# tyfeld/MMaDA-Parallel

Hardware: AMD Instinct MI355X
Metric: images/sec (512x512, 64 img + 128 text steps) MMaDA-Parallel-A 8B (higher is better)
Workload: dtype bf16

## Files before the change

mmada_parallel_amd/build.py:

```python
from __future__ import annotations

import os
import shutil
import subprocess
import sys
from concurrent.futures import ThreadPoolExecutor

HERE = os.path.dirname(os.path.abspath(__file__))
ROOT = os.path.dirname(HERE)
CSRC = os.path.join(HERE, "csrc")
OBJ = os.path.join(CSRC, "_obj")
LIB_NAME = "libmmada_mi355x.so"
LIB_PATH = os.path.join(HERE, LIB_NAME)
SOURCES = ["gemm.hip", "gemm8.hip", "attention.hip", "elementwise.hip", "sampler.hip", "vq_decoder.hip", "graph.hip", "tp_comm.hip", "probe.hip", "api.hip"]
HEADERS = ["exports.map", "common.h", "kernels.h", "gemm_epilogue.h", "handle.h", "attention.h", os.path.join("..", "..", "include", "mmada_mi355x.h")]
FLAGS = ["--offload-arch=gfx950", "-O3", "-std=c++17", "-fPIC", "-fvisibility=hidden", "-fvisibility-inlines-hidden", "-Wno-unused-result"]
UNIT_FLAGS = {"attention.hip": ["-fno-slp-vectorize", "-fno-honor-nans"]}


def _hipcc() -> str:
    for cand in (os.environ.get("HIPCC"), shutil.which("hipcc"), "/opt/rocm/bin/hipcc"):
        if cand and os.path.exists(cand):
            return cand
    raise RuntimeError("hipcc not found (set HIPCC or install ROCm)")


def needs_build() -> bool:
    if not os.path.exists(LIB_PATH):
        return True
    t = os.path.getmtime(LIB_PATH)
    deps = [os.path.join(CSRC, s) for s in SOURCES + HEADERS]
    return any(os.path.getmtime(d) > t for d in deps)


def _run(cmd):
    proc = subprocess.run(cmd, capture_output=True, text=True)
    if proc.returncode != 0:
        raise RuntimeError("hipcc failed:\n" + " ".join(cmd) + "\n" + proc.stdout + proc.stderr)
    return proc.stdout


def compile_objects(out_dir: str, extra_flags=(), force: bool = False, verbose: bool = False, jobs: int = 0):
    os.makedirs(out_dir, exist_ok=True)
    hdr_t = max(os.path.getmtime(os.path.join(CSRC, h)) for h in HEADERS)
    todo, objs = [], []
    for src in SOURCES:
        obj = os.path.join(out_dir, src.replace(".hip", ".o"))
        objs.append(obj)
        sp = os.path.join(CSRC, src)
        if force or not os.path.exists(obj) or os.path.getmtime(obj) < max(hdr_t, os.path.getmtime(sp)):
            todo.append([_hipcc(), *FLAGS, *UNIT_FLAGS.get(src, []), *extra_flags, "-c", sp, "-o", obj])
    if verbose:
        for c in todo:
            print(" ".join(c))
    with ThreadPoolExecutor(max_workers=jobs or min(len(todo) or 1, os.cpu_count() or 4)) as ex:
        list(ex.map(_run, todo))
    return objs


def verify_isa() -> None:
    tools = os.path.join(ROOT, "tools")
    if not os.path.exists(os.path.join(tools, "isa_check.py")):
        print("build: tools/isa_check.py not found, compiled-code checks skipped", file=sys.stderr)
        return
    if tools not in sys.path:
        sys.path.insert(0, tools)
    import isa_check

    with ThreadPoolExecutor(max_workers=2) as ex:
        asm8, asma = ex.map(isa_check.device_asm, ["gemm8.hip", "attention.hip"])
    errors = []
    errors += isa_check.check_gemm8(asm8)[1]
    errors += isa_check.check_gemm8_rowstat(asm8)[1]
    errors += isa_check.check_attention(asma)[1]
    if errors:
        raise RuntimeError("compiled-code checks failed (tools/isa_check.py):\n" + "\n".join(errors))


def build(force: bool = False, verbose: bool = False, verify: bool = False) -> str:
    if not force and not needs_build():
        return LIB_PATH
    with ThreadPoolExecutor(max_workers=2) as ex:
        chk = ex.submit(verify_isa) if verify else None
        objs = compile_objects(OBJ, force=force, verbose=verbose)
        _run([_hipcc(), "--offload-arch=gfx950", "-shared", "-fPIC", "-Wl,--version-script=" + os.path.join(CSRC, "exports.map"), *objs,
              "-o", LIB_PATH + ".tmp"])
        if chk is not None:
            try:
                chk.result()
            except Exception:
                for o in objs + [LIB_PATH + ".tmp"]:
                    if os.path.exists(o):
                        os.remove(o)
                raise
    os.replace(LIB_PATH + ".tmp", LIB_PATH)
    return LIB_PATH


if __name__ == "__main__":
    print(build(force="--force" in sys.argv, verbose=True, verify="--verify" in sys.argv))
```

mmada_parallel_amd/csrc/api.hip:

```cpp
#include <algorithm>
#include <cstdarg>
#include <cstdio>
#include <cstdlib>
#include <cstring>
#include <cmath>
#include <utility>
#include <vector>

#include "../../include/mmada_mi355x.h"
#include "handle.h"
#include "gemm_epilogue.h"

static thread_local char g_err[1024] = "";

int mm_fail(const char* fmt, ...) {
    va_list ap;
    va_start(ap, fmt);
    vsnprintf(g_err, sizeof(g_err), fmt, ap);
    va_end(ap);
    return 1;
}

extern "C" {

// ... 146 lines not shown
int mmada_embed(mmada_handle* h, const int64_t* ids, int B, int L, void* stream) {
    if (!h || !ids) return mm_fail("mmada_embed: null argument");
    hipStream_t s = (hipStream_t)stream;
    if (check_bound(h)) return 1;
    if (apply_carve(h, B, L, s)) return 1;
    h->cur_W = 0; h->cur_beg = 0; h->Mcur = h->M;
    h->xn_is_final = false;
    h->xn_is_layer0 = true;
    return launch_embed(ids, h->wte, h->x, B, L, h->Lp, h->cfg.d_model, h->cfg.vocab, s, h->layers[0].attn_norm, h->xn,
                        h->cfg.rms_eps);
}

}

GemmArgs qkv_args(const mmada_handle* h, int layer, int m0, int rows) {
    const int d = h->cfg.d_model;
    GemmArgs g = gemm_bt_args(h->xn + (size_t)m0 * d, h->layers[layer].wqkv, nullptr, rows, (h->hq_l + 2 * h->hkv_l) * 128, d, 0);
    g.m_base = m0;
    g.q = h->q; g.k = h->k; g.vT = h->vT; g.rope_cos = h->rope_cos; g.rope_sin = h->rope_sin;
    g.Lp = h->Lp; g.Lkv = h->Lkv; g.Hq = h->hq_l; g.Hkv = h->hkv_l;
    if (const CacheSlot* cc = h->cc) {
        g.k = cc->K(layer); g.vT = cc->vT(layer); g.Lkv = cc->Lkv;
        g.pos_map = h->cc_pos; g.Lq = h->Lkv; g.q_pos_shift = h->cc_qshift;
    }
    return g;
}

GemmArgs gate_up_args(const mmada_handle* h, int layer, int m0, int rows) {
    const int d = h->cfg.d_model;
    return gemm_bt_args(h->xn + (size_t)m0 * d, h->layers[layer].wgu, h->hbuf + (size_t)m0 * h->f_l, rows, 2 * h->f_l, d, h->f_l);
}

GemmArgs attn_out_args(const mmada_handle* h, int layer, int m0, int rows) {
    const int d = h->cfg.d_model, K = h->hq_l * 128;
    return gemm_bt_args(h->att + (size_t)m0 * K, h->layers[layer].wo, h->y + (size_t)m0 * d, rows, d, K, d);
}

GemmArgs down_args(const mmada_handle* h, int layer, int m0, int rows) {
    const int d = h->cfg.d_model;
    return gemm_bt_args(h->hbuf + (size_t)m0 * h->f_l, h->layers[layer].wdown, h->y + (size_t)m0 * d, rows, d, h->f_l, d);
}

int block_attention(mmada_handle* h, int layer, hipStream_t s, int wbeg, int W) {
    const CacheSlot* cc = h->cc;
    const double rows = W ? (double)h->B * W : (double)h->B * h->L;
    ProfScope p(h, layer, 1, 4.0 * h->hq_l * rows * (cc ? cc->L : h->L) * 128.0, s);
    if (cc)
        return launch_attention(h->q, cc->K(layer), cc->vT(layer), h->att, h->B, h->hq_l, h->hkv_l, cc->L, h->Lp, cc->Lkv, h->Lp,
                                h->hq_l * 128, s, 0, h->Lkv);
    if (W)
        return launch_attention(h->q, h->k, h->vT, h->att, h->B, h->hq_l, h->hkv_l, h->L, wbeg + W, h->Lkv, W, h->hq_l * 128, s,
                                wbeg);
    return launch_attention(h->q, h->k, h->vT, h->att, h->B, h->hq_l, h->hkv_l, h->L, h->Lp, h->Lkv, h->Lp, h->hq_l * 128, s);
}

static int run_blocks(mmada_handle* h, void* stream) {
    for (int i = 0; i < h->cfg.n_layers; ++i)
        if (mmada_attn_partial(h, i, stream) || mmada_mlp_partial(h, i, stream)) return 1;
    return 0;
}

extern "C" {

int mmada_attn_partial(mmada_handle* h, int layer, void* stream) {
    if (!h || h->M == 0) return mm_fail("mmada_attn_partial: call mmada_embed first");
    if (layer < 0 || layer >= h->cfg.n_layers) return mm_fail("mmada_attn_partial: bad layer");
    hipStream_t s = (hipStream_t)stream;
    const int d = h->cfg.d_model;
    if (layer == 0 && h->xn_is_layer0) {
        h->xn_is_layer0 = false;
    } else if (launch_rmsnorm(h->x, h->layers[layer].attn_norm, h->xn, h->M, d, h->cfg.rms_eps, s)) return 1;
    const GemmArgs g = qkv_args(h, layer, 0, h->M);
    const double rows = (double)h->B * h->L;
    {
        ProfScope p(h, layer, 0, 2.0 * rows * g.N * g.K, s);
        if (launch_gemm(EPI_QKV, g, s)) return 1;
    }
    int wbeg = 0, wend = 0, W = 0;
    if (!h->cc && layer == h->cfg.n_layers - 1 && h->win_end > h->win_beg) {
        if (h->win_end > h->L) return mm_fail("forward: consumed rows [%d,%d) exceed L=%d", h->win_beg, h->win_end, h->L);
        wbeg = h->win_beg & ~31;
        wend = std::min((h->win_end + 7) & ~7, h->Lp);
        W = wend - wbeg;
        if (W >= h->Lp) { wbeg = 0; W = 0; }
    }
    if (block_attention(h, layer, s, wbeg, W)) return 1;
    const int Mo = W ? h->B * W : h->M;
    const double orows = W ? (double)h->B * W : rows;
    GemmArgs o = attn_out_args(h, layer, 0, Mo);
    o.resid = h->x; o.ldr = d; o.resid_mod = h->cfg.tp_size; o.resid_rank = h->cfg.tp_rank;
    if (W) { o.rwin = W; o.rlp = h->Lp; o.rbeg = wbeg; }
    {
        ProfScope p(h, layer, 2, 2.0 * orows * o.N * o.K, s);
        if (launch_gemm(EPI_RESID, o, s)) return 1;
    }
    std::swap(h->x, h->y);
    if (W) { h->cur_W = W; h->cur_beg = wbeg; h->Mcur = Mo; }
    return 0;
}

int mmada_mlp_partial(mmada_handle* h, int layer, void* stream) {
    if (!h || h->M == 0) return mm_fail("mmada_mlp_partial: call mmada_embed first");
    if (layer < 0 || layer >= h->cfg.n_layers) return mm_fail("mmada_mlp_partial: bad layer");
    hipStream_t s = (hipStream_t)stream;
    const int d = h->cfg.d_model;
    if (launch_rmsnorm(h->x, h->layers[layer].ff_norm, h->xn, h->Mcur, d, h->cfg.rms_eps, s)) return 1;
    const GemmArgs g = gate_up_args(h, layer, 0, h->Mcur);
    const double rows = h->cur_W ? (double)h->Mcur : (double)h->B * h->L;
    {
        ProfScope p(h, layer, 3, 2.0 * rows * g.N * g.K, s);
        if (launch_gemm(EPI_SWIGLU, g, s)) return 1;
    }
    GemmArgs o = down_args(h, layer, 0, h->Mcur);
    o.resid = h->x; o.ldr = d; o.resid_mod = h->cfg.tp_size; o.resid_rank = h->cfg.tp_rank;
    {
        ProfScope p(h, layer, 4, 2.0 * rows * o.N * o.K, s);
        if (launch_gemm(EPI_RESID, o, s)) return 1;
    }
    std::swap(h->x, h->y);
    return 0;
}

int mmada_profile_begin(mmada_handle* h, int layer) {
    if (!h) return mm_fail("mmada_profile_begin: null handle");
    for (auto& r : h->prof) h->prof_pool.push_back({r.a, r.b});
    h->prof.clear();
    h->prof_layer = layer;
    return 0;
}

int mmada_profile_end(mmada_handle* h, int32_t* count_out, double* ms_out, double* flops_out) {
    if (!h || !count_out || !ms_out || !flops_out) return mm_fail("mmada_profile_end: null argument");
    for (int i = 0; i < 5; ++i) { count_out[i] = 0; ms_out[i] = 0.0; flops_out[i] = 0.0; }
    for (auto& r : h->prof) {
        MM_CHECK_HIP(hipEventSynchronize(r.b));
        float ms = 0.f;
        MM_CHECK_HIP(hipEventElapsedTime(&ms, r.a, r.b));
        count_out[r.kind] += 1; ms_out[r.kind] += ms; flops_out[r.kind] += r.flops;
        h->prof_pool.push_back({r.a, r.b});
    }
    h->prof.clear();
    h->prof_layer = -1;
    return 0;
}

}

static struct {
    std::atomic<int> gemm_config{-2};
    std::atomic<int> gemm_silu_lut{-1};
    std::atomic<int> gemm_short_tiles{-1};
    std::atomic<int> gemm_tile_order{-1};
    std::atomic<int> attention_form{-1};
    std::atomic<int> probe_variant{0};
    std::atomic<int> tp_allow_single_rank{0};
} g_switches;

static int env_int(const char* name, int fallback) {
    const char* e = getenv(name);
    return e ? atoi(e) : fallback;
}
static int env_flag(const char* name) {
    const char* e = getenv(name);
    return e && e[0] == '0' ? 0 : 1;
}

Switches switches() {
    static const Switches env = {env_int("MMADA_GEMM_CFG", -1), env_flag("MMADA_GEMM_SILU_LUT"), env_flag("MMADA_GEMM_SHORT_TILES"),
                                 env_int("MMADA_GEMM_TILE_ORDER", 0), env_int("MMADA_ATTN_FORM", 1), 0, 0};
    const int cfg = g_switches.gemm_config, lut = g_switches.gemm_silu_lut, shrt = g_switches.gemm_short_tiles,
              order = g_switches.gemm_tile_order, form = g_switches.attention_form;
    return {cfg == -2 ? env.gemm_config : cfg, lut < 0 ? env.gemm_silu_lut : lut, shrt < 0 ? env.gemm_short_tiles : shrt,
            order < 0 ? env.gemm_tile_order : order, form < 0 ? env.attention_form : form, g_switches.probe_variant,
            g_switches.tp_allow_single_rank};
}

extern "C" {

int mmada_set_option(const char* name, int value) {
    if (!name) return mm_fail("mmada_set_option: null name");
    static const struct { const char* name; std::atomic<int>* field; bool flag; } table[] = {
        {"gemm_config", &g_switches.gemm_config, false},
        {"gemm_silu_lut", &g_switches.gemm_silu_lut, true},
        {"gemm_short_tiles", &g_switches.gemm_short_tiles, true},
        {"gemm_tile_order", &g_switches.gemm_tile_order, false},
        {"attention_form", &g_switches.attention_form, false},
        {"probe_variant", &g_switches.probe_variant, false},
        {"tp_allow_single_rank", &g_switches.tp_allow_single_rank, true},
    };
    for (const auto& o : table)
        if (!strcmp(name, o.name)) {
            o.field->store(o.flag ? value != 0 : value);
            return 0;
        }
    return mm_fail("mmada_set_option: unknown option '%s'", name);
}

int mmada_gemm_swiglu_bt(const void* A, const void* W, void* C, int M, int N, int K, void* stream) {
    if (!A || !W || !C || M <= 0 || N <= 0 || K <= 0 || N % 64) return mm_fail("mmada_gemm_swiglu_bt: bad argument");
    return launch_gemm(EPI_SWIGLU, gemm_bt_args((const bf16_t*)A, (const bf16_t*)W, (bf16_t*)C, M, N, K, N / 2), (hipStream_t)stream);
}

int mmada_gemm_plan(int M, int N, int K) { return gemm_plan_code(M, N, K); }
int mmada_attention_plan(int pairs, int groups, int keys) {
    if (pairs <= 0 || groups <= 0 || keys <= 0) return mm_fail("mmada_attention_plan: bad argument"), -1;
    return attention_chunks(pairs, groups, keys);
}

int mmada_probe_f2bf(const float* in, uint16_t* out, int64_t n, void* stream) {
    if (!in || !out || n < 0) return mm_fail("mmada_probe_f2bf: bad argument");
    return launch_f2bf_probe(in, out, (long long)n, (hipStream_t)stream);
}

size_t mmada_mfma_probe_bytes(void) { return (size_t)64 * 8 * 16 * 64 * 16; }

int mmada_mfma_probe(const void* data, void* sink, int iters, int launches, void* stream, double* tflops_out, double* ms_out) {
    if (!data || !sink || iters <= 0 || launches <= 0) return mm_fail("mmada_mfma_probe: bad argument");
    return launch_mfma_probe((const bf16_t*)data, (float*)sink, iters, launches, (hipStream_t)stream, tflops_out, ms_out);
}

void* mmada_stream_ptr(mmada_handle* h) { return h ? (void*)h->x : nullptr; }
size_t mmada_stream_bytes(const mmada_handle* h) { return h ? (size_t)h->Mcur * h->cfg.d_model * 2 : 0; }

int mmada_forward_body(mmada_handle* h, const int64_t* ids, int B, int L, void* stream) {
    if (!h) return mm_fail("mmada_forward_body: null handle");
    if (h->cfg.tp_size != 1 || tp_comm_connected(h)) {
        if (!h->tp)
            return mm_fail("mmada_forward_body: tp_size=%d needs a connected collective (mmada_comm_create + "
                           "mmada_comm_connect_*) or the host-issued all-reduce of the segment API", h->cfg.tp_size);
        if (mmada_embed(h, ids, B, L, stream)) return 1;
        return tp_forward_body(h, (hipStream_t)stream);
    }
    if (mmada_embed(h, ids, B, L, stream)) return 1;
    return run_blocks(h, stream);
}

static void slot_layout(const mmada_handle* h, int B, int L, CacheSlot& c) {
    c.B = B; c.L = L; c.Lp = ceil_to(L, 8); c.Lkv = ceil_to(L, 64);
    c.kv_bytes = align_up((size_t)B * h->hkv_l * c.Lkv * 128 * 2, 256);
    c.layer_stride = 2 * c.kv_bytes;
    c.bytes = (size_t)h->cfg.n_layers * c.layer_stride + align_up((size_t)B * c.Lp * h->cfg.d_model * 2, 256);
}

size_t mmada_cache_bytes(const mmada_handle* h, int B, int L) {
    if (!h || B <= 0 || L <= 0) return 0;
    CacheSlot c;
    slot_layout(h, B, L, c);
    return c.bytes;
}

int mmada_cache_bind(mmada_handle* h, int slot, void* mem, size_t bytes, int B, int L, void* stream) {
    if (!h) return mm_fail("mmada_cache_bind: null handle");
    if (slot < 0 || slot >= MMADA_CACHE_SLOTS) return mm_fail("mmada_cache_bind: slot %d outside [0,%d)", slot, MMADA_CACHE_SLOTS);
    if (!mem) {
        h->slots[slot] = CacheSlot{};
        return 0;
    }
    if (h->cfg.tp_size != 1 && !tp_comm_connected(h))
        return mm_fail("mmada_cache_bind: tp_size=%d needs the library's exchange connected (mmada_comm_create + mmada_comm_connect_*)", h->cfg.tp_size);
    if (B <= 0 || L <= 0 || L > h->cfg.max_seq) return mm_fail("mmada_cache_bind: bad shape B=%d L=%d", B, L);
    if (((uintptr_t)mem) & 255) return mm_fail("mmada_cache_bind: memory must be 256-byte aligned");
    CacheSlot c;
    slot_layout(h, B, L, c);
    if (bytes < c.bytes) return mm_fail("mmada_cache_bind: %zu bytes given, %zu needed", bytes, c.bytes);
    c.mem = (char*)mem;
    MM_CHECK_HIP(hipMemsetAsync(mem, 0, c.bytes, (hipStream_t)stream));
    h->slots[slot] = c;
    return 0;
}

int mmada_forward_cached(mmada_handle* h, int slot, const int64_t* ids, const int32_t* pos, int B, int L, int Tc,
                         int q_pos_from_map, void* stream) {
    if (!h || !ids) return mm_fail("mmada_forward_cached: null argument");
    if (slot < 0 || slot >= MMADA_CACHE_SLOTS || !h->slots[slot].mem) return mm_fail("mmada_forward_cached: slot %d is not bound", slot);
    const CacheSlot& c = h->slots[slot];
    if (c.B != B || c.L != L) return mm_fail("mmada_forward_cached: slot holds B=%d L=%d, call has B=%d L=%d", c.B, c.L, B, L);
    const bool tp = h->cfg.tp_size != 1 || tp_comm_connected(h);
    if (tp && !tp_comm_connected(h)) return mm_fail("mmada_forward_cached: tp_size=%d needs the library's exchange connected", h->cfg.tp_size);
    if (!pos) Tc = L;
    if (Tc <= 0 || Tc > L) return mm_fail("mmada_forward_cached: Tc=%d outside (0,%d]", Tc, L);
    hipStream_t s = (hipStream_t)stream;
    if (check_bound(h)) return 1;
    if (apply_carve(h, B, L, s)) return 1;
    if (pos) {
        h->L = Tc; h->Lp = ceil_to(Tc, 8); h->Lkv = ceil_to(Tc, 64); h->M = B * h->Lp;
        if (launch_expand_pos(pos, h->posmap, B, Tc, h->Lp, L, s)) { h->M = 0; return 1; }
    }
    h->cur_W = 0; h->cur_beg = 0; h->Mcur = h->M;
    h->xn_is_final = false;
    h->xn_is_layer0 = true;
    const int d = h->cfg.d_model;
    if (launch_embed(ids, h->wte, h->x, B, h->L, h->Lp, d, h->cfg.vocab, s, h->layers[0].attn_norm, h->xn, h->cfg.rms_eps)) {
        h->M = 0;
        return 1;
    }
    h->cc = &c;
    h->cc_pos = pos ? h->posmap : nullptr;
    h->cc_qshift = (pos && !q_pos_from_map) ? L - Tc : -1;
    const int rc = tp ? tp_forward_body(h, s) : run_blocks(h, stream);
    h->cc = nullptr; h->cc_pos = nullptr; h->cc_qshift = -1;
    if (rc) { h->M = 0; return 1; }
    bf16_t* xfin = c.xfin(h->cfg.n_layers);
    const bf16_t* fin = tp ? h->xn : h->x;
    h->slots[slot].normalized = tp;
    if (pos) {
        if (launch_scatter_rows(fin, xfin, h->posmap, h->M, h->Lp, c.Lp, d, s)) { h->M = 0; return 1; }
    } else {
        MM_CHECK_HIP(hipMemcpyAsync(xfin, fin, (size_t)h->M * d * 2, hipMemcpyDeviceToDevice, s));
    }
    h->xn_is_final = false;
    h->M = 0;
    return 0;
}

int mmada_cache_head_rows(mmada_handle* h, int slot, const int32_t* rows, int R, int col_begin, int col_end,
                          void* logits_out, void* stream) {
    if (!h || !rows || !logits_out) return mm_fail("mmada_cache_head_rows: null argument");
    if (slot < 0 || slot >= MMADA_CACHE_SLOTS || !h->slots[slot].mem) return mm_fail("mmada_cache_head_rows: slot %d is not bound", slot);
    const CacheSlot& c = h->slots[slot];
    if (R <= 0) return 0;
    if (R > c.B * c.L) return mm_fail("mmada_cache_head_rows: R=%d exceeds B*L=%d", R, c.B * c.L);
    if (col_begin < 0 || col_end > h->cfg.vocab || col_begin >= col_end) return mm_fail("mmada_cache_head_rows: bad column range");
    hipStream_t s = (hipStream_t)stream;
    const int d = h->cfg.d_model;
    bf16_t* xg;
    if (h->M != 0) {
        if ((size_t)R > (size_t)h->B * h->L)
            return mm_fail("mmada_cache_head_rows: %d rows do not fit the resident forward's gather buffer (%d x %d rows); "
                           "ask for fewer rows per call", R, h->B, h->L);
        xg = h->xg;
    } else {
        const Carve cv = carve_for(h, c.B, c.L);
        if (!h->ws || cv.total > h->ws_bytes) return mm_fail("mmada_cache_head_rows: workspace too small (%zu needed)", cv.total);
        xg = (bf16_t*)(h->ws + cv.xg);
    }
    if (c.normalized) {
        if (tp_gather_rows(c.xfin(h->cfg.n_layers), rows, R, c.L, c.Lp, d, c.B * c.L, xg, s)) return 1;
    } else if (launch_rmsnorm_gather(c.xfin(h->cfg.n_layers), h->ln_f, xg, rows, R, c.L, c.Lp, d, h->cfg.rms_eps, s, 0, c.B * c.L))
// ... 195 lines not shown
```

mmada_parallel_amd/csrc/gemm8.hip:

```cpp
#include "gemm_epilogue.h"

namespace {

using namespace gemm_detail;

constexpr int BK = 64;

#define G8_SB() __builtin_amdgcn_sched_barrier(0)
#define G8_BARRIER()                            \
    do {                                        \
        G8_SB();                                \
        asm volatile("s_barrier" ::: "memory"); \
        G8_SB();                                \
    } while (0)

typedef __attribute__((address_space(3))) const bf16x8* lds_frag_ptr;
#pragma clang diagnostic push
#pragma clang diagnostic ignored "-Wint-to-pointer-cast"
#pragma clang diagnostic ignored "-Wint-to-void-pointer-cast"
MM_DEVICE lds_frag_ptr lds_frag(int byte_off) { return (lds_frag_ptr)(uint32_t)byte_off; }
MM_DEVICE lptr_t lds_at(int byte_off) { return (lptr_t)(uint32_t)byte_off; }
#pragma clang diagnostic pop

MM_DEVICE void dma16(const char* sbase, unsigned& voff, int lds_byte) {
    const int m0v = __builtin_amdgcn_readfirstlane(lds_byte);
    asm volatile("s_mov_b32 m0, %2\n\tglobal_load_lds_dwordx4 %1, %0" ::"s"(sbase), "v"(voff), "s"(m0v) : "memory");
}

template <int N>
MM_DEVICE void wait_vm() {
    G8_SB();
    asm volatile("s_waitcnt vmcnt(%0)" ::"n"(N) : "memory");
    G8_SB();
}

template <int BM_, int BN_, int WM_, int WN_, int SW_, int OPT_ = 0>
struct Gemm8 {
    static constexpr int BM = BM_, BN = BN_, WM = WM_, WN = WN_, SW = SW_, OPT = OPT_;
    static constexpr int TM = BM / WM, TN = BN / WN, FM = TM / 16, FN = TN / 16;
    static constexpr int FA0 = (FM + 1) / 2, FA1 = FM / 2, FB = FN / 2;
    static constexpr int A_BYTES = BM * 128, B_BYTES = BN * 128, W_BASE = 2 * A_BYTES, LDS = 2 * (A_BYTES + B_BYTES);
    static_assert(A_BYTES + TM * 128 <= 65536 && B_BYTES + TN * 128 <= 65536, "second buffer within the ds_read immediate");
    static constexpr int NPA0 = WM * FA0 * 2, NPA1 = WM * FA1 * 2, NPB = WN * FB * 2;
    static constexpr int RA0 = NPA0 % 8, RA1 = NPA1 % 8;
    static constexpr int REM = RA0 ? RA0 : RA1;
    static constexpr int NB = NPB / 8;
    static_assert(WM * WN == 8 && TM % 16 == 0 && TN % 32 == 0 && FA1 >= 1, "wave tile");
    static constexpr bool CAN_DROP = WM == 2 && FA1 >= 2 && BM == 320;
    static constexpr int SHORT_BM = BM - 16;
    static_assert(NPB % 8 == 0 && (RA0 == 0 || RA1 == 0 || RA0 == RA1) && NPA0 <= 24 && NPA1 <= 24, "piece split");
    static_assert(LDS + SiluLut::BYTES <= 160 * 1024, "LDS (K-tile buffers + the SwiGLU epilogue's SiLU table)");

    const char* Ab;
    const char* Wb;
    const char* Zb;
    unsigned alane, wlane;
    unsigned arow[2][3], wrow[2][2];
    bool azero[2][3];
    int alds[2][3], wlds[2][2];
    int ra[2], rb[2];
    const char* lut_src;
    int lut_wave;
    bf16x8 af[FA0][2], bf0[FB][2], bf1[FB][2];
    f32x4 acc[FM][FN];

    MM_DEVICE void init(const GemmArgs& g, int m0, int n0, int wave, int lane) {
        Ab = (const char*)(g.A + (size_t)((OPT & 64) ? 0 : m0) * g.lda);
        Wb = (const char*)(g.W + (size_t)((OPT & 64) ? 0 : n0) * g.ldw);
        Zb = (const char*)g.zero_row;
        const int wm = wave / WN, wn = wave % WN;
        const int prow = lane >> 3, psw = ((wave & 1) * 4 + (prow >> 1)) & 7;
        alane = (unsigned)prow * (unsigned)(g.lda * 2) + (((lane & 7) ^ psw) << 4);
        wlane = (unsigned)prow * (unsigned)(g.ldw * 2) + (((lane & 7) ^ psw) << 4);
        const int mrem = g.M - m0, nrem = g.N - n0;
#pragma unroll
        for (int h = 0; h < 2; ++h) {
            const int fa = h ? FA1 : FA0, npa = h ? NPA1 : NPA0;
#pragma unroll
            for (int i = 0; i < 3; ++i) {
                const int p = min(wave + 8 * i, npa - 1);
                const int row0 = (p / (fa * 2)) * TM + (h ? FA0 * 16 : 0) + (p % (fa * 2)) * 8;
                azero[h][i] = Zb != nullptr && row0 >= mrem;
                arow[h][i] = azero[h][i] ? 0u : (unsigned)min(row0, mrem - 8) * (unsigned)(g.lda * 2);
                alds[h][i] = row0 * 128;
            }
#pragma unroll
            for (int i = 0; i < NB; ++i) {
                const int p = wave + 8 * i;
                const int row0 = (p / (FB * 2)) * TN + h * FB * 16 + (p % (FB * 2)) * 8;
                wrow[h][i] = (unsigned)min(row0, nrem - 8) * (unsigned)(g.ldw * 2);
                wlds[h][i] = W_BASE + row0 * 128;
            }
        }
        const int frow = lane & 15, fq = lane >> 4, sw = (frow >> 1) & 7;
#pragma unroll
        for (int kk = 0; kk < 2; ++kk) {
            const int lanepart = frow * 128 + (((kk * 4 + fq) ^ sw) << 4);
            ra[kk] = wm * TM * 128 + lanepart;
            rb[kk] = W_BASE + wn * TN * 128 + lanepart;
            asm volatile("" : "+v"(ra[kk]), "+v"(rb[kk]));
        }
#pragma unroll
        for (int i = 0; i < FM; ++i)
#pragma unroll
            for (int j = 0; j < FN; ++j) acc[i][j] = f32x4{0.f, 0.f, 0.f, 0.f};
        if (OPT & 16) {
            bf16x8 junk;
#pragma unroll
            for (int e = 0; e < 8; ++e) junk[e] = (__bf16)(0.37f + 0.01f * (float)((lane * 7 + e * 13) & 63));
#pragma unroll
            for (int kk = 0; kk < 2; ++kk) {
#pragma unroll
                for (int i = 0; i < FA0; ++i) af[i][kk] = junk;
#pragma unroll
                for (int j = 0; j < FB; ++j) { bf0[j][kk] = junk; bf1[j][kk] = junk; }
            }
        }
    }

    template <int B, int H, int NA>
    MM_DEVICE void stage_a(int kt) {
        if (OPT & 8) return;
#pragma unroll
        for (int i = 0; i < NA; ++i) {
            const char* src = (azero[H][i] ? Zb : Ab + arow[H][i]) + (size_t)kt * (BK * 2);
            dma16(src, alane, B * A_BYTES + alds[H][i]);
        }
    }
    template <int B, int H>
    MM_DEVICE void stage_w(int kt) {
        if (OPT & 8) return;
#pragma unroll
        for (int i = 0; i < NB; ++i) {
            const char* src = Wb + wrow[H][i] + (size_t)kt * (BK * 2);
            dma16(src, wlane, B * B_BYTES + wlds[H][i]);
        }
    }
    template <int B, int H, int DROP = 0>
    MM_DEVICE void read_a() {
        if (OPT & 16) return;
#pragma unroll
        for (int mi = 0; mi < (H ? FA1 - DROP : FA0); ++mi)
#pragma unroll
            for (int kk = 0; kk < 2; ++kk) af[mi][kk] = *lds_frag(ra[kk] + B * A_BYTES + ((H ? FA0 * 16 : 0) + mi * 16) * 128);
    }
    template <int B, int H>
    MM_DEVICE void read_b(bf16x8 (&bf)[FB][2]) {
        if (OPT & 16) return;
#pragma unroll
        for (int nj = 0; nj < FB; ++nj)
#pragma unroll
            for (int kk = 0; kk < 2; ++kk) bf[nj][kk] = *lds_frag(rb[kk] + B * B_BYTES + (H * FB * 16 + nj * 16) * 128);
    }
    template <int H, int NH, bool SWAP, int DROP = 0>
    MM_DEVICE void mma(bf16x8 (&bf)[FB][2]) {
#pragma unroll
        for (int kk = 0; kk < 2; ++kk)
#pragma unroll
            for (int mi = 0; mi < (H ? FA1 - DROP : FA0); ++mi)
#pragma unroll
                for (int nj = 0; nj < FB; ++nj) {
                    f32x4& c = acc[(H ? FA0 : 0) + mi][NH * FB + nj];
                    if (OPT & 4) { asm volatile("" : "+v"(c) : "v"(af[mi][kk]), "v"(bf[nj][kk])); continue; }
                    c = SWAP ? __builtin_amdgcn_mfma_f32_16x16x32_bf16(bf[nj][kk], af[mi][kk], c, 0, 0, 0)
                             : __builtin_amdgcn_mfma_f32_16x16x32_bf16(af[mi][kk], bf[nj][kk], c, 0, 0, 0);
                }
    }


    template <int B, int NA0, int NA1, int TAIL, bool SWAP, int DROP>
    MM_DEVICE void tile(int kt) {
        constexpr int FOUR = NA0 + NA1 + 2 * NB;
        if (TAIL < 2) stage_w<B ^ 1, 1>(kt + 1);
        read_a<B, 0>();
        read_b<B, 0>(bf0);
        if (TAIL < 2) wait_vm<FOUR>(); else wait_vm<NA1>();
        G8_BARRIER();
        mma<0, 0, SWAP>(bf0);
        G8_BARRIER();
        if (TAIL < 2) stage_a<B ^ 1, 1, NA1>(kt + 1);
        read_b<B, 1>(bf1);
        if (TAIL < 2) wait_vm<FOUR>(); else wait_vm<0>();
        G8_BARRIER();
        mma<0, 1, SWAP>(bf1);
        G8_BARRIER();
        if (TAIL == 0) stage_a<B, 0, NA0>(kt + 2);
        read_a<B, 1, DROP>();
        G8_BARRIER();
        mma<1, 1, SWAP, DROP>(bf1);
        G8_BARRIER();
        if (TAIL == 0) stage_w<B, 0>(kt + 2);
        if (TAIL == 0) wait_vm<FOUR>();
        else if (TAIL == 1) wait_vm<NB + NA1>();
        G8_BARRIER();
        mma<1, 0, SWAP, DROP>(bf0);
        G8_BARRIER();
    }


    template <int B, int NA0, int NA1, int TAIL, bool SWAP, int DROP>
    MM_DEVICE void tile_bal(int kt) {
        constexpr int FOUR = NA0 + NA1 + 2 * NB;
        bf16x8(&F)[FB][2] = B ? bf1 : bf0;
        bf16x8(&S)[FB][2] = B ? bf0 : bf1;
        if (TAIL < 2) stage_w<B ^ 1, 1>(kt + 1);
        read_a<B, 0>();
        if (TAIL < 2) wait_vm<FOUR>(); else wait_vm<NA1>();
        G8_BARRIER();
        mma<0, 0, SWAP>(F);
        G8_BARRIER();
        if (TAIL < 2) stage_a<B ^ 1, 1, NA1>(kt + 1);
        read_b<B, 1>(S);
        if (TAIL < 2) wait_vm<FOUR>(); else wait_vm<0>();
        G8_BARRIER();
        mma<0, 1, SWAP>(S);
        G8_BARRIER();
        if (TAIL == 0) stage_w<B, 0>(kt + 2);
        read_a<B, 1, DROP>();
        if (TAIL == 0) wait_vm<FOUR>();
        else if (TAIL == 1) wait_vm<NA0 + NB + NA1>();
        G8_BARRIER();
        mma<1, 1, SWAP, DROP>(S);
        G8_BARRIER();
        if (TAIL == 0) stage_a<B, 0, NA0>(kt + 2);
        if (TAIL < 2) read_b<B ^ 1, 0>(S);
        if (TAIL == 0) wait_vm<FOUR>();
        else if (TAIL == 1) wait_vm<NB + NA1>();
        G8_BARRIER();
        mma<1, 0, SWAP, DROP>(F);
        G8_BARRIER();
    }

    template <int NA0, int NA1, bool SWAP, int DROP>
    MM_DEVICE void run(int nk, int grp) {
        constexpr bool BAL = (OPT & 2) != 0;
        wait_vm<0>();
        if (lut_src) {
            unsigned lane16 = (unsigned)__builtin_amdgcn_mbcnt_hi(~0u, __builtin_amdgcn_mbcnt_lo(~0u, 0u)) * 16u;
#pragma unroll
            for (int i = 0; i < 2; ++i) {
                const int p = lut_wave + 8 * i;
                if (p < SiluLut::PIECES) dma16(lut_src + p * 1024, lane16, LDS + p * 1024);
            }
        }
        stage_a<0, 0, NA0>(0); stage_w<0, 0>(0); stage_w<0, 1>(0); stage_a<0, 1, NA1>(0);
        if (BAL) { stage_w<1, 0>(1); stage_a<1, 0, NA0>(1); }
        else { stage_a<1, 0, NA0>(1); stage_w<1, 0>(1); }
        wait_vm<NA0 + NA1 + 2 * NB>();
        G8_BARRIER();
        if (BAL) read_b<0, 0>(bf0);
        if (grp == 1) G8_BARRIER();
        if ((OPT & 1) && grp == 1) __builtin_amdgcn_s_setprio(1);
        if constexpr (BAL) {
            for (int kt = 0; kt + 2 < nk; kt += 2) {
                tile_bal<0, NA0, NA1, 0, SWAP, DROP>(kt);
                tile_bal<1, NA0, NA1, 0, SWAP, DROP>(kt + 1);
            }
            int one = 1;
            asm volatile("" : "+s"(one));
#pragma nounroll
            for (int t = 0; t < one; ++t) {
                tile_bal<0, NA0, NA1, 1, SWAP, DROP>(nk - 2);
                tile_bal<1, NA0, NA1, 2, SWAP, DROP>(nk - 1);
            }
        } else {
            for (int kt = 0; kt + 2 < nk; kt += 2) {
                tile<0, NA0, NA1, 0, SWAP, DROP>(kt);
                tile<1, NA0, NA1, 0, SWAP, DROP>(kt + 1);
            }
            int one = 1;
            asm volatile("" : "+s"(one));
#pragma nounroll
            for (int t = 0; t < one; ++t) {
                tile<0, NA0, NA1, 1, SWAP, DROP>(nk - 2);
                tile<1, NA0, NA1, 2, SWAP, DROP>(nk - 1);
            }
        }
        if (grp == 0) G8_BARRIER();
    }
};

template <int EPI, class G>
__global__ __launch_bounds__(512, 2) void gemm8_kernel(GemmArgs g) {
    const int wave = __builtin_amdgcn_readfirstlane(threadIdx.x >> 6);
    const int ntm = (g.M + G::BM - 1) / G::BM, ntn = (g.N + G::BN - 1) / G::BN;
    int mt, nt;
    tile_coords_g(xcd_remap(blockIdx.x, gridDim.x), ntm, ntn, g.tile_gm, g.tile_gn, mt, nt);
    const bool short_tiles = G::CAN_DROP && g.row_drop != 0;
    const bool short_tile = short_tiles && mt < ntm - 1;
    const int m0 = mt * (short_tiles ? G::SHORT_BM : G::BM), n0 = nt * G::BN;
    const int m_lim = short_tile ? m0 + G::SHORT_BM : g.M;
    const bool drop = short_tile && wave / G::WN == G::WM - 1;
    G k;
    const bool use_lut = EPI == EPI_SWIGLU && g.silu_lut != nullptr;
    const int lut_lds = use_lut ? G::LDS : -1;
    k.init(g, m0, n0, wave, threadIdx.x & 63);
    k.lut_src = use_lut ? (const char*)g.silu_lut : nullptr;
    k.lut_wave = wave;
    const int nk = g.K / BK;
    const bool extra = G::REM != 0 && wave < G::REM;
    const bool swap = G::SW == 1 || (G::SW == 2 && !qkv_wave_is_v(g, n0 + (wave % G::WN) * G::TN));
    constexpr int NA0 = G::NPA0 / 8, NA1 = G::NPA1 / 8, XA0 = NA0 + (G::RA0 ? 1 : 0), XA1 = NA1 + (G::RA1 ? 1 : 0);
#define G8_PATH1(A0, A1, SWP, DRP)                                                                  \
    do {                                                                                            \
        k.template run<A0, A1, SWP, DRP>(nk, wave >> 2);                                            \
        const int lane = __builtin_amdgcn_mbcnt_hi(~0u, __builtin_amdgcn_mbcnt_lo(~0u, 0u));        \
        if (SWP) gemm_epilogue_t<EPI, G::TM, G::TN, G::WN>(g, m0, n0, k.acc, wave, lane, m_lim, lut_lds); \
        else gemm_epilogue<EPI, G::TM, G::TN, G::WN>(g, m0, n0, k.acc, wave, lane, m_lim);               \
    } while (0)
#define G8_PATH(A0, A1, SWP)                                                                        \
    do {                                                                                            \
        if constexpr (G::CAN_DROP) {                                                                \
            if (drop) G8_PATH1(A0, A1, SWP, 1);                                                     \
            else G8_PATH1(A0, A1, SWP, 0);                                                          \
        } else G8_PATH1(A0, A1, SWP, 0);                                                            \
    } while (0)
    if (G::SW != 0 && swap) {
        if (extra) G8_PATH(XA0, XA1, true);
        else G8_PATH(NA0, NA1, true);
    } else if (G::SW != 1) {
        if (extra) G8_PATH(XA0, XA1, false);
        else G8_PATH(NA0, NA1, false);
    }
#undef G8_PATH
#undef G8_PATH1
    gemm_publish(g, wave);
}

template <int EPI, class G>
int launch_cfg8(const GemmArgs& g, const Switches& sw, hipStream_t s) {
    auto fn = gemm8_kernel<EPI, G>;
    static MmOncePerDevice attr_set;
    constexpr int LDS_BYTES = G::LDS + (EPI == EPI_SWIGLU ? SiluLut::BYTES : 0);
    MM_ONCE_PER_DEVICE(attr_set, MM_CHECK_HIP(hipFuncSetAttribute((const void*)fn, hipFuncAttributeMaxDynamicSharedMemorySize, LDS_BYTES)));
    const int ntm = (g.M + G::BM - 1) / G::BM, ntn = (g.N + G::BN - 1) / G::BN;
    GemmArgs ga = g;
    ga.row_drop = G::CAN_DROP && sw.gemm_short_tiles && ntm >= 2 && (ntm - 1) * G::SHORT_BM + G::BM >= g.M ? 1 : 0;
    constexpr int DEF_GM = (G::BM == 320 && G::BN == 256) ? 4 : 0, DEF_GN = (G::BM == 320 && G::BN == 256) ? 8 : 1024 / G::BN;
    const int order = sw.gemm_tile_order;
    ga.tile_gm = order > 0 ? order / 100 : DEF_GM;
    ga.tile_gn = order > 0 && order % 100 > 0 ? order % 100 : DEF_GN;
    hipLaunchKernelGGL(fn, dim3(ntm * ntn), dim3(512), LDS_BYTES, s, ga);
    MM_CHECK_HIP(hipGetLastError());
    return 0;
}

template <int EPI>
int launch_epi8(int cfg, const GemmArgs& g, const Switches& sw, hipStream_t s) {
    constexpr int SW = EPI == EPI_QKV ? 2 : 1;
    if constexpr (EPI == EPI_ROWSTAT) {
        switch (cfg) {
            case GEMM8_320x256: return launch_cfg8<EPI, Gemm8<320, 256, 2, 4, SW, 2>>(g, sw, s);
            case GEMM8_256x256: return launch_cfg8<EPI, Gemm8<256, 256, 2, 4, SW, 2>>(g, sw, s);
            case GEMM8_160x256: return launch_cfg8<EPI, Gemm8<160, 256, 2, 4, SW, 2>>(g, sw, s);
        }
        return mm_fail("gemm8: configuration %d has no row-statistics epilogue", cfg);
    } else
    switch (cfg) {
        case GEMM8_320x256: return launch_cfg8<EPI, Gemm8<320, 256, 2, 4, SW, 2>>(g, sw, s);
        case GEMM8_256x256: return launch_cfg8<EPI, Gemm8<256, 256, 2, 4, SW, 2>>(g, sw, s);
        case GEMM8_160x256: return launch_cfg8<EPI, Gemm8<160, 256, 2, 4, SW, 2>>(g, sw, s);
        case GEMM8_320x128: return launch_cfg8<EPI, Gemm8<320, 128, 4, 2, SW, 2>>(g, sw, s);
#ifdef MMADA_TUNE
        case 4: return launch_cfg8<EPI, Gemm8<320, 256, 2, 4, SW, 3>>(g, sw, s);
        case 5: return launch_cfg8<EPI, Gemm8<320, 128, 4, 2, SW, 0>>(g, sw, s);
        case 6: return launch_cfg8<EPI, Gemm8<320, 256, 2, 4, SW, 0>>(g, sw, s);
        case 7: return launch_cfg8<EPI, Gemm8<256, 256, 2, 4, SW, 0>>(g, sw, s);
        case 8: return launch_cfg8<EPI, Gemm8<160, 256, 2, 4, SW, 0>>(g, sw, s);
        case 9: return launch_cfg8<EPI, Gemm8<320, 256, 2, 4, SW, 4>>(g, sw, s);
        case 10: return launch_cfg8<EPI, Gemm8<320, 256, 2, 4, SW, 8>>(g, sw, s);
        case 11: return launch_cfg8<EPI, Gemm8<320, 256, 2, 4, SW, 16>>(g, sw, s);
        case 12: return launch_cfg8<EPI, Gemm8<320, 256, 2, 4, SW, 24>>(g, sw, s);
        case 13: return launch_cfg8<EPI, Gemm8<320, 256, 2, 4, SW, 20>>(g, sw, s);
        case 14: return launch_cfg8<EPI, Gemm8<320, 256, 2, 4, SW, 84>>(g, sw, s);
        case 15: return launch_cfg8<EPI, Gemm8<320, 256, 2, 4, SW, 64>>(g, sw, s);
#endif
    }
    return mm_fail("gemm8: unknown configuration %d", cfg);
}

}

bool gemm8_supports(const GemmArgs& g) {
    return g.K % 128 == 0 && g.K >= 256 && g.M % 8 == 0 && g.N % 8 == 0 && g.M >= 8 && g.N >= 8 &&
           (long long)g.lda * 2 * 328 < (1ll << 31) && (long long)g.ldw * 2 * 264 < (1ll << 31) &&
           g.ldc % 8 == 0 && (g.resid == nullptr || g.ldr % 8 == 0) && ((uintptr_t)g.C & 15) == 0 && ((uintptr_t)g.resid & 15) == 0;
}

int launch_gemm8(int epi, int cfg, const GemmArgs& g, const Switches& sw, hipStream_t s) {
    if (!gemm8_supports(g)) return mm_fail("gemm8: unsupported shape M=%d N=%d K=%d", g.M, g.N, g.K);
    switch (epi) {
        case EPI_STORE: return launch_epi8<EPI_STORE>(cfg, g, sw, s);
        case EPI_RESID: return launch_epi8<EPI_RESID>(cfg, g, sw, s);
        case EPI_SWIGLU: return launch_epi8<EPI_SWIGLU>(cfg, g, sw, s);
        case EPI_QKV: return launch_epi8<EPI_QKV>(cfg, g, sw, s);
        case EPI_ROWSTAT: return launch_epi8<EPI_ROWSTAT>(cfg, g, sw, s);
    }
    return mm_fail("gemm8: bad epilogue %d", epi);
}
```

mmada_parallel_amd/csrc/kernels.h:

```cpp
#pragma once
#include <hip/hip_runtime.h>
#include <stdint.h>
#include "common.h"

enum GemmEpilogue { EPI_STORE = 0, EPI_RESID = 1, EPI_SWIGLU = 2, EPI_QKV = 3, EPI_ROWSTAT = 4 };

struct GemmArgs {
    const bf16_t* A;
    const bf16_t* W;
    bf16_t* C;
    int M, N, K;
    int lda, ldw, ldc;
    const bf16_t* resid;
    int ldr;
    int resid_mod, resid_rank;
    int rwin, rlp, rbeg;
    const bf16_t* zero_row;
    bf16_t* q;
    bf16_t* k;
    bf16_t* vT;
    const float* rope_cos;
    const float* rope_sin;
    int Lp, Lkv, Hq, Hkv;
    int publish;
    int m_base;
    const int32_t* pos_map;
    int Lq, q_pos_shift;
    const uint16_t* silu_lut;
    int row_drop;
    int tile_gm, tile_gn;
};

int launch_gemm(int epi, const GemmArgs& g, hipStream_t s);

struct RowStatArgs {
    float4* part;
    float* tx;
    const int64_t* target;
    int rows, ld, col0;
};
static inline __host__ __device__ RowStatArgs rowstat_args(const GemmArgs& g) {
    return RowStatArgs{(float4*)g.C, (float*)g.resid, (const int64_t*)g.pos_map, g.rwin, g.rlp, g.rbeg};
}
static inline void set_rowstat_args(GemmArgs& g, const RowStatArgs& r) {
    g.C = (bf16_t*)r.part; g.resid = (const bf16_t*)r.tx; g.pos_map = (const int32_t*)r.target;
    g.ldc = 8; g.ldr = 8;
    g.rwin = r.rows; g.rlp = r.ld; g.rbeg = r.col0;
}

static inline GemmArgs gemm_bt_args(const bf16_t* A, const bf16_t* W, bf16_t* C, int M, int N, int K, int ldc) {
    GemmArgs g{};
    g.A = A; g.W = W; g.C = C;
    g.M = M; g.N = N; g.K = K;
    g.lda = K; g.ldw = K; g.ldc = ldc;
    return g;
}

struct Switches {
    int gemm_config, gemm_silu_lut, gemm_short_tiles, gemm_tile_order, attention_form, probe_variant, tp_allow_single_rank;
};
Switches switches();

size_t head_rowstat_bytes(int R, int N);
int launch_head_rowstat(const bf16_t* A, const bf16_t* W, int R, int N, int K, int col0, const int64_t* targets, void* part,
                        float* logprob, float* lse, int32_t* argmax, float* vmax, hipStream_t s);

int launch_embed(const int64_t* ids, const bf16_t* wte, bf16_t* x, int B, int L, int Lp, int d, int vocab, hipStream_t s,
                 const bf16_t* norm_w = nullptr, bf16_t* xn = nullptr, float eps = 0.f);
int launch_rmsnorm(const bf16_t* x, const bf16_t* w, bf16_t* out, int rows, int d, float eps, hipStream_t s);
int launch_rmsnorm_gather(const bf16_t* x, const bf16_t* w, bf16_t* out, const int32_t* rows, int R, int L, int row_stride,
                          int d, float eps, hipStream_t s, int row_off = 0, int nflat = 0);
int launch_rope_table(float* cos_t, float* sin_t, const float* inv_freq_dev, int max_seq, hipStream_t s);
int launch_unpad_rows(const bf16_t* x, bf16_t* out, int B, int L, int Lp, int d, hipStream_t s);
int launch_iota_rows(int32_t* rows, int n, hipStream_t s);
int launch_expand_pos(const int32_t* pos, int32_t* posmap, int B, int Tc, int Lp, int L, hipStream_t s);
int launch_scatter_rows(const bf16_t* src, bf16_t* dst, const int32_t* posmap, int M, int Lp, int Lp_dst, int d, hipStream_t s);
int launch_pack_qkv(const bf16_t* wq, const bf16_t* wk, const bf16_t* wv, bf16_t* out, int d, int Hq, int Hkv, int tp_rank,
                    int tp_size, hipStream_t s);
int launch_pack_gate_up(const bf16_t* gate, const bf16_t* up, bf16_t* out, int d, int F, int tp_rank, int tp_size,
                        hipStream_t s);
int launch_pack_cols(const bf16_t* w, bf16_t* out, int rows, int cols, int tp_rank, int tp_size, hipStream_t s);
int launch_pad_heads(const bf16_t* in, bf16_t* out, int BH, int L, int Lkv, hipStream_t s);
int launch_transpose_v(const bf16_t* v, bf16_t* vT, int BH, int L, int Lkv, hipStream_t s);
int launch_lfq_gather(const int64_t* idx, void* out, int B, int N, int nbits, int f32, hipStream_t s);

int launch_attention(const bf16_t* q, const bf16_t* k, const bf16_t* vT, bf16_t* out, int B, int Hq, int Hkv, int L,
                     int Lq_rows, int Lkv, int out_row_stride_per_batch, int ld_out, hipStream_t s, int q_begin = 0,
                     int Lq_alloc = 0);

int attention_chunks(int pairs, int groups, int keys);

struct TextStat { float lmax; int32_t arg; double sum; };
int launch_text_stats_partial(const bf16_t* logits, int B, int T, int Vl, int ld, int col_off, const int64_t* ids, int L,
                              int text_start, int mask_id, TextStat* out, hipStream_t s);
int launch_text_commit(const void* scratch, int B, int T, int64_t* ids, int L, int text_start, const int32_t* k, hipStream_t s);
int launch_text_select(const bf16_t* logits, const bf16_t* noisy, const bf16_t* unc, float text_cfg, const int32_t* x0_in,
                       int B, int T, int V, int ld, int64_t* ids, int L, int text_start, const int32_t* k, void* scratch,
                       int mask_id, hipStream_t s, const float* rand_conf = nullptr);
int launch_image_probs(const bf16_t* cond, const bf16_t* ut, const bf16_t* ui, int B, int N, int CB, float cfg_scale,
                       float cfg_img, bf16_t* probs_out, int32_t* argmax_out, bf16_t* pmax_out, int mvar, hipStream_t s);
int launch_image_commit(int64_t* ids, int B, int L, const int32_t* pos_map, int N, const int32_t* sampled_in,
                        const bf16_t* p_in, const bf16_t* noise, float remask_temp, const int32_t* mask_len_sched,
                        int mask_id, int text_vocab, int codebook, int mvar, hipStream_t s);

int launch_f2bf_probe(const float* in, bf16_t* out, long long n, hipStream_t s);
int launch_mfma_probe(const bf16_t* data, float* sink, int iters, int launches, hipStream_t s, double* tflops_out, double* ms_out);
```

Measured before the change: 0.1422.

## Add software-pipelined K loop for 256x256 and 160x256 bf16 GEMM tiles

Adds a tile_pipe path to the Gemm8 kernel for the 256x256 and 160x256 configurations. It splits each K tile into four MFMA quarters and interleaves the LDS fragment reads for the next quarter between MFMAs using sched_group_barrier. It also stages one more W block ahead in the prologue and keeps a second A-fragment register set. The aim is to hide LDS read latency behind matrix math. In exchange it uses more VGPRs, which could lower occupancy. The path is on by default through the MMADA_GEMM_PIPE flag, and an ISA check was added for it.

```diff
diff --git a/mmada_parallel_amd/build.py b/mmada_parallel_amd/build.py
--- a/mmada_parallel_amd/build.py
+++ b/mmada_parallel_amd/build.py
@@ -71,6 +71,7 @@
         asm8, asma = ex.map(isa_check.device_asm, ["gemm8.hip", "attention.hip"])
     errors = []
     errors += isa_check.check_gemm8(asm8)[1]
+    errors += isa_check.check_gemm8_pipe(asm8)[1]
     errors += isa_check.check_gemm8_rowstat(asm8)[1]
     errors += isa_check.check_attention(asma)[1]
     if errors:
diff --git a/mmada_parallel_amd/csrc/api.hip b/mmada_parallel_amd/csrc/api.hip
--- a/mmada_parallel_amd/csrc/api.hip
+++ b/mmada_parallel_amd/csrc/api.hip
@@ -322,6 +322,7 @@
     std::atomic<int> gemm_short_tiles{-1};
     std::atomic<int> gemm_tile_order{-1};
     std::atomic<int> attention_form{-1};
+    std::atomic<int> gemm_pipe{-1};
     std::atomic<int> probe_variant{0};
     std::atomic<int> tp_allow_single_rank{0};
 } g_switches;
@@ -337,12 +338,12 @@
 
 Switches switches() {
     static const Switches env = {env_int("MMADA_GEMM_CFG", -1), env_flag("MMADA_GEMM_SILU_LUT"), env_flag("MMADA_GEMM_SHORT_TILES"),
-                                 env_int("MMADA_GEMM_TILE_ORDER", 0), env_int("MMADA_ATTN_FORM", 1), 0, 0};
+                                 env_int("MMADA_GEMM_TILE_ORDER", 0), env_int("MMADA_ATTN_FORM", 1), 0, 0, env_flag("MMADA_GEMM_PIPE")};
     const int cfg = g_switches.gemm_config, lut = g_switches.gemm_silu_lut, shrt = g_switches.gemm_short_tiles,
-              order = g_switches.gemm_tile_order, form = g_switches.attention_form;
+              order = g_switches.gemm_tile_order, form = g_switches.attention_form, pipe = g_switches.gemm_pipe;
     return {cfg == -2 ? env.gemm_config : cfg, lut < 0 ? env.gemm_silu_lut : lut, shrt < 0 ? env.gemm_short_tiles : shrt,
             order < 0 ? env.gemm_tile_order : order, form < 0 ? env.attention_form : form, g_switches.probe_variant,
-            g_switches.tp_allow_single_rank};
+            g_switches.tp_allow_single_rank, pipe < 0 ? env.gemm_pipe : pipe};
 }
 
 extern "C" {
@@ -354,6 +355,7 @@
         {"gemm_silu_lut", &g_switches.gemm_silu_lut, true},
         {"gemm_short_tiles", &g_switches.gemm_short_tiles, true},
         {"gemm_tile_order", &g_switches.gemm_tile_order, false},
+        {"gemm_pipe", &g_switches.gemm_pipe, true},
         {"attention_form", &g_switches.attention_form, false},
         {"probe_variant", &g_switches.probe_variant, false},
         {"tp_allow_single_rank", &g_switches.tp_allow_single_rank, true},
diff --git a/mmada_parallel_amd/csrc/gemm8.hip b/mmada_parallel_amd/csrc/gemm8.hip
--- a/mmada_parallel_amd/csrc/gemm8.hip
+++ b/mmada_parallel_amd/csrc/gemm8.hip
@@ -34,8 +34,13 @@
     G8_SB();
 }
 
+template <int N, bool ON>
+struct Gemm8PipeFrags { bf16x8 af1[N][2]; };
+template <int N>
+struct Gemm8PipeFrags<N, false> {};
+
 template <int BM_, int BN_, int WM_, int WN_, int SW_, int OPT_ = 0>
-struct Gemm8 {
+struct Gemm8 : Gemm8PipeFrags<BM_ / WM_ / 32, (OPT_ & 32) != 0> {
     static constexpr int BM = BM_, BN = BN_, WM = WM_, WN = WN_, SW = SW_, OPT = OPT_;
     static constexpr int TM = BM / WM, TN = BN / WN, FM = TM / 16, FN = TN / 16;
     static constexpr int FA0 = (FM + 1) / 2, FA1 = FM / 2, FB = FN / 2;
@@ -231,9 +236,83 @@
         G8_BARRIER();
     }
 
+    template <int B, int H, int NF>
+    MM_DEVICE void read_a_to(bf16x8 (&a)[NF][2]) {
+        static_assert(NF == (H ? FA1 : FA0), "fragment set of that A half");
+#pragma unroll
+        for (int mi = 0; mi < NF; ++mi)
+#pragma unroll
+            for (int kk = 0; kk < 2; ++kk) a[mi][kk] = *lds_frag(ra[kk] + B * A_BYTES + ((H ? FA0 * 16 : 0) + mi * 16) * 128);
+    }
+    template <int H, int NH, bool SWAP, int NF>
+    MM_DEVICE void mma_from(bf16x8 (&a)[NF][2], bf16x8 (&bf)[FB][2]) {
+#pragma unroll
+        for (int kk = 0; kk < 2; ++kk)
+#pragma unroll
+            for (int mi = 0; mi < NF; ++mi)
+#pragma unroll
+                for (int nj = 0; nj < FB; ++nj) {
+                    f32x4& c = acc[(H ? FA0 : 0) + mi][NH * FB + nj];
+                    c = SWAP ? __builtin_amdgcn_mfma_f32_16x16x32_bf16(bf[nj][kk], a[mi][kk], c, 0, 0, 0)
+                             : __builtin_amdgcn_mfma_f32_16x16x32_bf16(a[mi][kk], bf[nj][kk], c, 0, 0, 0);
+                }
+    }
+    template <int NM, int NR>
+    MM_DEVICE void pin_reads() {
+        static_assert(NR <= NM, "one read per MFMA gap");
+#pragma unroll
+        for (int i = 0; i < NR; ++i) {
+            __builtin_amdgcn_sched_group_barrier(0x008, 1, 0);
+            __builtin_amdgcn_sched_group_barrier(0x100, 1, 0);
+        }
+        if (NM > NR) __builtin_amdgcn_sched_group_barrier(0x008, NM - NR, 0);
+    }
+
+    template <int B, int NA0, int NA1, int TAIL, bool SWAP>
+    MM_DEVICE void tile_pipe(int kt) {
+        constexpr int FOUR = NA0 + NA1 + 2 * NB;
+        bf16x8(&F)[FB][2] = B ? bf1 : bf0;
+        bf16x8(&S)[FB][2] = B ? bf0 : bf1;
+        if (TAIL < 2) stage_a<B ^ 1, 1, NA1>(kt + 1);
+        asm volatile("s_waitcnt lgkmcnt(0)" ::: "memory");
+        if (TAIL < 2) wait_vm<FOUR>(); else wait_vm<0>();
+        G8_BARRIER();
+        mma_from<0, 0, SWAP>(af, F);
+        read_b<B, 1>(S);
+        pin_reads<FA0 * FB * 2, FB * 2>();
+        G8_BARRIER();
+        if (TAIL == 0) stage_w<B, 0>(kt + 2);
+        if (TAIL == 0) wait_vm<FOUR>();
+        else if (TAIL == 1) wait_vm<NA0 + NB + NA1>();
+        G8_BARRIER();
+        mma_from<0, 1, SWAP>(af, S);
+        read_a_to<B, 1>(this->af1);
+        pin_reads<FA0 * FB * 2, FA1 * 2>();
+        G8_BARRIER();
+        if (TAIL == 0) stage_a<B, 0, NA0>(kt + 2);
+        if (TAIL == 0) wait_vm<FOUR>();
+        else if (TAIL == 1) wait_vm<NB + NA1>();
+        G8_BARRIER();
+        mma_from<1, 1, SWAP>(this->af1, S);
+        G8_BARRIER();
+        if (TAIL == 0) stage_w<B, 1>(kt + 2);
+        if (TAIL < 2) read_b<B ^ 1, 0>(S);
+        if (TAIL == 0) wait_vm<FOUR>();
+        else if (TAIL == 1) wait_vm<NA1>();
+        G8_BARRIER();
+        mma_from<1, 0, SWAP>(this->af1, F);
+        if (TAIL < 2) {
+            read_a_to<B ^ 1, 0>(af);
+            pin_reads<FA1 * FB * 2, FA0 * 2>();
+        }
+        G8_BARRIER();
+    }
+
     template <int NA0, int NA1, bool SWAP, int DROP>
     MM_DEVICE void run(int nk, int grp) {
         constexpr bool BAL = (OPT & 2) != 0;
+        constexpr bool PIPE = (OPT & 32) != 0;
+        static_assert(!PIPE || (BAL && !CAN_DROP && (OPT & 28) == 0 && FA0 * 2 <= FA1 * FB * 2), "tile_pipe: balanced builds of the short tiles");
         wait_vm<0>();
         if (lut_src) {
             unsigned lane16 = (unsigned)__builtin_amdgcn_mbcnt_hi(~0u, __builtin_amdgcn_mbcnt_lo(~0u, 0u)) * 16u;
@@ -246,12 +325,26 @@
         stage_a<0, 0, NA0>(0); stage_w<0, 0>(0); stage_w<0, 1>(0); stage_a<0, 1, NA1>(0);
         if (BAL) { stage_w<1, 0>(1); stage_a<1, 0, NA0>(1); }
         else { stage_a<1, 0, NA0>(1); stage_w<1, 0>(1); }
+        if (PIPE) stage_w<1, 1>(1);
         wait_vm<NA0 + NA1 + 2 * NB>();
         G8_BARRIER();
         if (BAL) read_b<0, 0>(bf0);
+        if (PIPE) read_a_to<0, 0>(af);
         if (grp == 1) G8_BARRIER();
         if ((OPT & 1) && grp == 1) __builtin_amdgcn_s_setprio(1);
-        if constexpr (BAL) {
+        if constexpr (PIPE) {
+            for (int kt = 0; kt + 2 < nk; kt += 2) {
+                tile_pipe<0, NA0, NA1, 0, SWAP>(kt);
+                tile_pipe<1, NA0, NA1, 0, SWAP>(kt + 1);
+            }
+            int one = 1;
+            asm volatile("" : "+s"(one));
+#pragma nounroll
+            for (int t = 0; t < one; ++t) {
+                tile_pipe<0, NA0, NA1, 1, SWAP>(nk - 2);
+                tile_pipe<1, NA0, NA1, 2, SWAP>(nk - 1);
+            }
+        } else if constexpr (BAL) {
             for (int kt = 0; kt + 2 < nk; kt += 2) {
                 tile_bal<0, NA0, NA1, 0, SWAP, DROP>(kt);
                 tile_bal<1, NA0, NA1, 0, SWAP, DROP>(kt + 1);
@@ -358,8 +451,10 @@
     } else
     switch (cfg) {
         case GEMM8_320x256: return launch_cfg8<EPI, Gemm8<320, 256, 2, 4, SW, 2>>(g, sw, s);
-        case GEMM8_256x256: return launch_cfg8<EPI, Gemm8<256, 256, 2, 4, SW, 2>>(g, sw, s);
-        case GEMM8_160x256: return launch_cfg8<EPI, Gemm8<160, 256, 2, 4, SW, 2>>(g, sw, s);
+        case GEMM8_256x256: return sw.gemm_pipe ? launch_cfg8<EPI, Gemm8<256, 256, 2, 4, SW, 34>>(g, sw, s)
+                                                : launch_cfg8<EPI, Gemm8<256, 256, 2, 4, SW, 2>>(g, sw, s);
+        case GEMM8_160x256: return sw.gemm_pipe ? launch_cfg8<EPI, Gemm8<160, 256, 2, 4, SW, 34>>(g, sw, s)
+                                                : launch_cfg8<EPI, Gemm8<160, 256, 2, 4, SW, 2>>(g, sw, s);
         case GEMM8_320x128: return launch_cfg8<EPI, Gemm8<320, 128, 4, 2, SW, 2>>(g, sw, s);
 #ifdef MMADA_TUNE
         case 4: return launch_cfg8<EPI, Gemm8<320, 256, 2, 4, SW, 3>>(g, sw, s);
diff --git a/mmada_parallel_amd/csrc/kernels.h b/mmada_parallel_amd/csrc/kernels.h
--- a/mmada_parallel_amd/csrc/kernels.h
+++ b/mmada_parallel_amd/csrc/kernels.h
@@ -57,7 +57,7 @@
 }
 
 struct Switches {
-    int gemm_config, gemm_silu_lut, gemm_short_tiles, gemm_tile_order, attention_form, probe_variant, tp_allow_single_rank;
+    int gemm_config, gemm_silu_lut, gemm_short_tiles, gemm_tile_order, attention_form, probe_variant, tp_allow_single_rank, gemm_pipe;
 };
 Switches switches();
 
```

New measurement: 0.1423 (median of 6 runs). No clear change (+0.1%).
